# ACCtools/alignasm

Measured on AMD Instinct MI355X. Metric: contigs_per_sec, higher is better.
Workload: dtype int64

## Files before the change

alignasm_amd/_abi.py:

```python
import ctypes as C

import numpy as np

AASM_N_PHASES = 16
PHASE_NAMES = ["sort", "pairs", "edges", "revcsr", "sptree", "fwd", "heap", "enum", "select", "gather", "heap_prep", "topo", "misc", "cs", "final", "chain"]

AASM_OK = 0
AASM_E_INVAL, AASM_E_NODEVICE, AASM_E_HIP, AASM_E_NOMEM = -1, -2, -3, -4
AASM_E_OVERFLOW, AASM_E_INTERNAL, AASM_E_PARSE, AASM_E_IO = -5, -6, -7, -8

AASM_READ_DEVICE_RANGES, AASM_READ_H_WEAK_HASH, AASM_READ_H_FEW_BLOCKS = 1, 0x100, 0x200
AASM_READ_ROW_COLS, AASM_READ_TEXT_ON_DEVICE = 2, 4

DEBUG_POISON_SIG = (C.c_int, [C.c_int])

_IN_ARRAYS = [
    ("ctg_rec_off", np.int64), ("qry_str", np.int64), ("qry_end", np.int64), ("ref_str", np.int64),
    ("ref_end", np.int64), ("qry_total", np.int64), ("ref_chr", np.int32), ("aln_fwd", np.uint8),
    ("map_qul", np.uint8), ("rec_rng_off", np.int64), ("rng_qry_l", np.int64), ("rng_qry_r", np.int64),
    ("rng_ref_l", np.int64),
]


class BatchIn(C.Structure):
    _fields_ = [("n_contigs", C.c_int64), ("n_records", C.c_int64), ("n_ranges", C.c_int64)] + [
        (name, C.c_void_p) for name, _ in _IN_ARRAYS
    ] + [("cs_text", C.c_void_p), ("rec_cs_off", C.c_void_p)]


class Opts(C.Structure):
    _fields_ = [
        ("max_paths", C.c_int32), ("non_skip_linkable", C.c_int32), ("device", C.c_int32),
        ("collect_timing", C.c_int32), ("keep_debug", C.c_int32), ("reserved", C.c_int32 * 3),
    ]


AASM_H0_SEQ_SELECT, AASM_H0_HEAP_MW_ALL, AASM_H0_HEAP_MW_NONE, AASM_H0_ENUM_HEAP, AASM_H0_ENUM_SMALL = 0x1, 0x2, 0x4, 0x8, 0x10
AASM_H0_GRID_ORDER, AASM_H0_CHAIN_MASK, AASM_H0_CHAIN_ALL, AASM_H0_CHAIN_NONE, AASM_H0_CHAIN_HALF = 0x20, 0xC0, 0x40, 0x80, 0xC0
AASM_H0_MW_MASK, AASM_H0_MW_INPUT_ORDER, AASM_H0_MW_SHIFT, AASM_H0_GRAPH_LAUNCHES = 0xFF00, 1, 8, 0x10000
AASM_H2_LAUNCH_FAILURE, AASM_H2_WRAP_DEVICES, AASM_H2_DIRTY_SCAN, AASM_H2_CHAIN_HDR_LOST, AASM_H2_CHAIN_DONE_LOST = 0x1, 0x2, 0x4, 0x8, 0x10
AASM_H2_CHAIN_OWN_QUEUE, AASM_H2_SMALL_ROOT_RING, AASM_H2_SORT_DEPTH_MASK, AASM_H2_SORT_DEPTH_SHIFT = 0x20, 0x40, 0xFF00, 8
HOOK_CONSTANTS = {k: v for k, v in globals().items() if k.startswith(("AASM_H0_", "AASM_H2_"))}
_flag = lambda bits: {False: 0, True: bits}
HOOKS = {
    "sequential_select": (0, _flag(AASM_H0_SEQ_SELECT)), "heap_waves": (0, {"auto": 0, "all": AASM_H0_HEAP_MW_ALL, "none": AASM_H0_HEAP_MW_NONE}),
    "enum_heap": (0, _flag(AASM_H0_ENUM_HEAP)), "enum_small": (0, _flag(AASM_H0_ENUM_SMALL)), "grid_order": (0, _flag(AASM_H0_GRID_ORDER)),
    "chain": (0, {"auto": 0, "all": AASM_H0_CHAIN_ALL, "none": AASM_H0_CHAIN_NONE, "half": AASM_H0_CHAIN_HALF}),
    "heap_input_order": (0, _flag(AASM_H0_MW_INPUT_ORDER << AASM_H0_MW_SHIFT)), "heap_block_waves": (0, {n: n << AASM_H0_MW_SHIFT for n in (0, 4, 8, 16)}),
    "graph_launches": (0, _flag(AASM_H0_GRAPH_LAUNCHES)), "test_max_contigs": (1, None),
    "test_inject_launch_failure": (2, _flag(AASM_H2_LAUNCH_FAILURE)), "wrap_devices": (2, _flag(AASM_H2_WRAP_DEVICES)), "test_dirty_scan": (2, _flag(AASM_H2_DIRTY_SCAN)),
    "test_chain_lost": (2, {0: 0, 1: AASM_H2_CHAIN_HDR_LOST, 2: AASM_H2_CHAIN_DONE_LOST}), "chain_own_queue": (2, _flag(AASM_H2_CHAIN_OWN_QUEUE)),
    "test_small_root_ring": (2, _flag(AASM_H2_SMALL_ROOT_RING)), "sort_depth_test": (2, {d: d << AASM_H2_SORT_DEPTH_SHIFT for d in range(256)}),
}


def make_opts(max_paths=10000, non_skip_linkable=False, device=0, timing=False, keep_debug=False, **hooks):
    o = Opts(int(max_paths), 1 if non_skip_linkable else 0, int(device), 1 if timing else 0, 1 if keep_debug else 0)
    for name, value in hooks.items():
        if name not in HOOKS:
            raise TypeError(f"unknown test hook {name!r}")
        word, table = HOOKS[name]
        if table is not None and value not in table:
            raise ValueError(f"test hook {name}={value!r}: not one of {sorted(table, key=str)}")
        o.reserved[word] |= int(value) if table is None else table[value]
    if hooks.get("heap_input_order") and hooks.get("heap_block_waves"):
        raise ValueError("heap_input_order and heap_block_waves set the same field")
    return o


class OutElem(C.Structure):
    _fields_ = [
        ("edited_qry_str", C.c_int64), ("edited_qry_end", C.c_int64), ("edited_ref_str", C.c_int64),
        ("edited_ref_end", C.c_int64), ("ctg_index", C.c_int32), ("is_alt_path", C.c_int32),
    ]


OUT_ELEM_DTYPE = np.dtype(
    [("qs", np.int64), ("qe", np.int64), ("rs", np.int64), ("re", np.int64), ("ctg_index", np.int32), ("is_alt", np.int32)]
)

_STAT_I64 = [
    "n_vertices", "n_pairs", "n_edges", "n_heap_nodes", "n_paths_found", "n_paths_converted",
# ... 240 lines not shown
```

alignasm_amd/csrc/aasm_gpu.hip:

```cpp
#include <hip/hip_runtime.h>
#include <initializer_list>

#include <atomic>
#include <chrono>
#include <functional>
#include <mutex>
#include <thread>
#include <fcntl.h>
#include <sys/mman.h>
#include <sys/stat.h>
#include <unistd.h>

#include "aasm_pipeline.h"
#include "aasm_ksw.h"
#include "aasm_cut.h"
#include "aasm_read.h"
#include "aasm_rows.h"
#include "aasm_paf.hpp"

namespace aasm {

__device__ inline int64_t xcd_bid(int64_t b, int64_t g, int on) {
    if (!on || g < 64) return b;
    const int64_t g8 = g & ~(int64_t)7;
// ... 186 lines not shown
    for (int64_t base = 0; base < n; base += 4096) {
        const int64_t i0 = base + (int64_t)threadIdx.x * 4;
        int64_t va[4], vb[4], sa = 0, sb = 0;
#pragma unroll
        for (int i = 0; i < 4; i++) { va[i] = (i0 + i < n) ? (int64_t)in_a[i0 + i] : 0; sa += va[i]; vb[i] = (in_b && i0 + i < n) ? (int64_t)in_b[i0 + i] : 0; sb += vb[i]; }
        const int64_t ia = scan_wave_incl(sa, lane), ib = scan_wave_incl(sb, lane);
        if (lane == 63) { sh_w[0][wv] = ia; sh_w[1][wv] = ib; }
        __syncthreads();
        int64_t oa = sh_carry[0], ob = sh_carry[1], ta = 0, tb = 0;
#pragma unroll
        for (int i = 0; i < 16; i++) { const int64_t xa = sh_w[0][i], xb = sh_w[1][i]; if (i < wv) { oa += xa; ob += xb; } ta += xa; tb += xb; }
        int64_t ra = oa + ia - sa, rb = ob + ib - sb;
#pragma unroll
        for (int i = 0; i < 4; i++) { if (i0 + i < n) { out_a[i0 + i] = ra; if (in_b) out_b[i0 + i] = rb; } ra += va[i]; rb += vb[i]; }
        __syncthreads();
        if (threadIdx.x == 0) { sh_carry[0] += ta; sh_carry[1] += tb; }
        __syncthreads();
    }
    if (threadIdx.x == 0) { out_a[n] = sh_carry[0]; if (in_b) out_b[n] = sh_carry[1]; }
}

struct ScalarSrc { const int64_t *p[12]; };
__global__ void aasm_read_scalars(ScalarSrc src, int n, int64_t *dst) {
    const int i = (int)threadIdx.x;
    if (i < n) __hip_atomic_store(dst + i, *src.p[i], __ATOMIC_RELAXED, __HIP_MEMORY_SCOPE_SYSTEM);
}

struct ArenaBlock { char *p; size_t cap, used; };

struct DevCtx {
    int device = -1;
    bool ready = false;
    hipStream_t stream = nullptr, side = nullptr, side2 = nullptr;
    hipEvent_t ev_fork, ev_join, ev_fork2, ev_join2, ev_fork_b;
    int64_t *d_scratch2 = nullptr;
    size_t d_scratch2_cap = 0;
    std::vector<ArenaBlock> blocks;
    int64_t *pinned = nullptr;
    int64_t *pinned_dev = nullptr;
    char *stage[2] = {nullptr, nullptr};
    int64_t *d_scratch = nullptr;
    size_t d_scratch_cap = 0;
    uint64_t generation = 0;
    std::atomic<int> input_arrived{0};
    std::mutex mu;
    hipEvent_t ev_b[AASM_N_PHASES], ev_e[AASM_N_PHASES], ev_t0, ev_t1;
    int n_events_made = 0;
    int n_events2 = 0;
    hipEvent_t *timing_event(int i) { return i < AASM_N_PHASES ? &ev_b[i] : i < 2 * AASM_N_PHASES ? &ev_e[i - AASM_N_PHASES] : i == 2 * AASM_N_PHASES ? &ev_t0 : &ev_t1; }
    bool events = false;
    size_t peak_bytes = 0;
    std::vector<hipEvent_t> export_events;
};

static void drain_exports(DevCtx &cx) {
    for (hipEvent_t e : cx.export_events) { (void)hipEventSynchronize(e); (void)hipEventDestroy(e); }
    cx.export_events.clear();
}
static DevCtx g_ctx[16];
static std::mutex g_init_mu;
static std::atomic<int64_t> g_n_range_splits{0}, g_n_device_mallocs{0}, g_n_stream_syncs{0}, g_n_read_slow_rows{0}, g_n_read_fallbacks{0}, g_n_read_containers{0};

static std::atomic<int> g_poison{0};
static inline int poison_byte() { return g_poison.load(std::memory_order_relaxed); }

static std::string hip_err(const char *what, hipError_t e) {
    return std::string(what) + ": " + hipGetErrorString(e);
}

static int ctx_init(int device) {
    if (device < 0 || device >= 16) { set_last_error("device ordinal out of range"); return AASM_E_INVAL; }
    std::lock_guard<std::mutex> lk(g_init_mu);
    DevCtx &cx = g_ctx[device];
    if (cx.ready) return AASM_OK;
    int n = 0;
    hipError_t e = hipGetDeviceCount(&n);
    if (e != hipSuccess || n <= 0) { set_last_error("no HIP device available (this library has no CPU fallback)"); return AASM_E_NODEVICE; }
    if (device >= n) { set_last_error("device ordinal beyond hipGetDeviceCount"); return AASM_E_NODEVICE; }
    if ((e = hipSetDevice(device)) != hipSuccess) { set_last_error(hip_err("hipSetDevice", e)); return AASM_E_NODEVICE; }
    auto fail = [&](const char *what, hipError_t err) {
        set_last_error(hip_err(what, err));
        if (cx.pinned) { hipHostFree(cx.pinned); cx.pinned = nullptr; }
        if (cx.n_events_made > 0) { hipEventDestroy(cx.ev_fork); }
        if (cx.n_events_made > 1) { hipEventDestroy(cx.ev_join); }
        for (int i = 2; i < cx.n_events_made; i++) hipEventDestroy(*cx.timing_event(i - 2));
        cx.n_events_made = 0;
        if (cx.n_events2 > 0) { hipEventDestroy(cx.ev_fork2); }
        if (cx.n_events2 > 1) { hipEventDestroy(cx.ev_join2); }
        if (cx.n_events2 > 2) { hipEventDestroy(cx.ev_fork_b); }
        cx.n_events2 = 0;
        if (cx.side2) { hipStreamDestroy(cx.side2); cx.side2 = nullptr; }
        if (cx.side) { hipStreamDestroy(cx.side); cx.side = nullptr; }
        if (cx.stream) { hipStreamDestroy(cx.stream); cx.stream = nullptr; }
        return AASM_E_NODEVICE;
    };
    if ((e = hipStreamCreateWithFlags(&cx.stream, hipStreamNonBlocking)) != hipSuccess) return fail("hipStreamCreate", e);
    if ((e = hipStreamCreateWithFlags(&cx.side, hipStreamNonBlocking)) != hipSuccess) return fail("hipStreamCreate", e);
    if ((e = hipStreamCreateWithFlags(&cx.side2, hipStreamNonBlocking)) != hipSuccess) return fail("hipStreamCreate", e);
    if ((e = hipEventCreateWithFlags(&cx.ev_fork2, hipEventDisableTiming)) != hipSuccess) return fail("hipEventCreate", e);
    cx.n_events2 = 1;
    if ((e = hipEventCreateWithFlags(&cx.ev_join2, hipEventDisableTiming)) != hipSuccess) return fail("hipEventCreate", e);
    cx.n_events2 = 2;
    if ((e = hipEventCreateWithFlags(&cx.ev_fork_b, hipEventDisableTiming)) != hipSuccess) return fail("hipEventCreate", e);
    cx.n_events2 = 3;
    if ((e = hipEventCreateWithFlags(&cx.ev_fork, hipEventDisableTiming)) != hipSuccess) return fail("hipEventCreate", e);
    cx.n_events_made = 1;
    if ((e = hipEventCreateWithFlags(&cx.ev_join, hipEventDisableTiming)) != hipSuccess) return fail("hipEventCreate", e);
    cx.n_events_made = 2;
    for (int i = 0; i < 2 * AASM_N_PHASES + 2; i++) {
        if ((e = hipEventCreate(cx.timing_event(i))) != hipSuccess) return fail("hipEventCreate", e);
        cx.n_events_made++;
    }
    if ((e = hipHostMalloc((void **)&cx.pinned, 64 * sizeof(int64_t), hipHostMallocMapped)) != hipSuccess) return fail("hipHostMalloc", e);
    std::memset(cx.pinned, 0, 64 * sizeof(int64_t));
    if ((e = hipHostGetDevicePointer((void **)&cx.pinned_dev, cx.pinned, 0)) != hipSuccess) return fail("hipHostGetDevicePointer", e);
    cx.events = true;
    cx.device = device;
    cx.ready = true;
    return AASM_OK;
}

struct GpuBackend {
    static constexpr bool host_emulation = false;
    DevCtx &cx;
    hipStream_t stream, main_stream;
    bool on_side = false, forked = false, forked2 = false;
    bool timing;
    bool fail = false, out_of_memory = false;
    bool phase_used[AASM_N_PHASES] = {false};
    size_t cur_block = 0, bytes = 0;
    std::map<std::string, std::pair<void *, size_t>> named;
    GpuBackend(DevCtx &c, hipStream_t s, bool t) : cx(c), stream(s), main_stream(s), timing(t) {
        drain_exports(cx);
        for (auto &b : cx.blocks) b.used = 0;
        cx.generation++;
    }
    struct Attach {};
    GpuBackend(DevCtx &c, hipStream_t s, Attach) : cx(c), stream(s), main_stream(s), timing(false) {}
    void hip_fail(const char *what, hipError_t e) { if (!fail) set_last_error(hip_err(what, e)); fail = true; }
    void *alloc(const char *name, size_t n) {
        n = (n + 255) & ~(size_t)255;
        while (cur_block < cx.blocks.size() && cx.blocks[cur_block].used + n > cx.blocks[cur_block].cap) cur_block++;
        if (cur_block >= cx.blocks.size()) {
            size_t have = 0;
            for (auto &b : cx.blocks) have += b.cap;
            size_t cap = have > ((size_t)1 << 30) ? have : ((size_t)1 << 30);
            if (cap < n) cap = n;
            char *p = nullptr;
            hipError_t e = hipMalloc((void **)&p, cap);
            g_n_device_mallocs++;
            if (e == hipErrorOutOfMemory && cap > n) { (void)hipGetLastError(); cap = n; e = hipMalloc((void **)&p, cap); g_n_device_mallocs++; }
            if (e != hipSuccess) {
                if (e == hipErrorOutOfMemory) { (void)hipGetLastError(); out_of_memory = true; if (!fail) set_last_error("out of device memory (workspace arena)"); fail = true; }
                else hip_fail("hipMalloc", e);
                return nullptr;
            }
            cx.blocks.push_back(ArenaBlock{p, cap, 0});
            cur_block = cx.blocks.size() - 1;
            if (const int pz = poison_byte()) {
// ... 111 lines not shown
    int64_t read_i64(const int64_t *p) { int64_t v = 0; read_i64s({p}, &v); return v; }
    void read_i64s(std::initializer_list<const int64_t *> ps, int64_t *out) {
        int n = 0;
        for (auto p : ps) { (void)p; out[n++] = 0; }
        flush_zero();
        if (fail) return;
        ScalarSrc src;
        int i = 0;
        for (auto p : ps) { if (i < 12) src.p[i] = p; i++; }
        for (int j = i; j < 12; j++) src.p[j] = nullptr;
        hipLaunchKernelGGL(aasm_read_scalars, dim3(1), dim3(64), 0, stream, src, n, cx.pinned_dev);
        hipError_t e = hipGetLastError();
        if (e == hipSuccess) e = hipStreamSynchronize(stream);
        g_n_stream_syncs++;
        if (e != hipSuccess) { hip_fail("scalar read-back", e); return; }
        if (scan_stalled()) return;
        for (i = 0; i < n; i++) out[i] = cx.pinned[i];
    }
    void d2h(void *dst, const void *src, size_t n) {
        flush_zero();
        if (fail || n == 0) return;
        hipError_t e = hipMemcpyAsync(dst, src, n, hipMemcpyDeviceToHost, stream);
        if (e == hipSuccess) e = hipStreamSynchronize(stream);
        if (e != hipSuccess) hip_fail("hipMemcpy D2H", e);
        scan_stalled();
    }
    void h2d(void *dst, const void *src, size_t n) {
        flush_zero();
        if (fail || n == 0) return;
        hipError_t e = hipMemcpyAsync(dst, src, n, hipMemcpyHostToDevice, stream);
        if (e != hipSuccess) hip_fail("hipMemcpy H2D", e);
    }
    void fork() { flush_zero(); if (fail) return; hipEventRecord(cx.ev_fork, main_stream); hipStreamWaitEvent(cx.side, cx.ev_fork, 0); forked = true; }
    void fork_again() { flush_zero(); if (fail) return; hipEventRecord(cx.ev_fork_b, main_stream); hipStreamWaitEvent(cx.side, cx.ev_fork_b, 0); forked = true; }
    void use_side(bool on) { flush_zero(); on_side = on; stream = on ? cx.side : main_stream; }
    void join() { flush_zero(); if (fail || !forked) return; hipEventRecord(cx.ev_join, cx.side); hipStreamWaitEvent(main_stream, cx.ev_join, 0); forked = false; }
    void fork2() { flush_zero(); if (fail) return; hipEventRecord(cx.ev_fork2, main_stream); hipStreamWaitEvent(cx.side2, cx.ev_fork2, 0); forked2 = true; }
    void use_side2(bool on) { flush_zero(); stream = on ? cx.side2 : main_stream; }
    void join2() { flush_zero(); if (fail || !forked2) return; hipEventRecord(cx.ev_join2, cx.side2); hipStreamWaitEvent(main_stream, cx.ev_join2, 0); forked2 = false; }
    void phase_begin(int ph) { flush_zero(); if (timing && !fail) { hipError_t e = hipEventRecord(cx.ev_b[ph], stream); if (e != hipSuccess) hip_fail("hipEventRecord", e); phase_used[ph] = true; } }
    void phase_end(int ph) { flush_zero(); if (timing && !fail) { hipError_t e = hipEventRecord(cx.ev_e[ph], stream); if (e != hipSuccess) hip_fail("hipEventRecord", e); } }
};

struct GraphGpu {
    hipStream_t stream;
    const char *entry;
    hipError_t e = hipSuccess;
    std::vector<void *> blocks;
    ~GraphGpu() { for (void *p : blocks) hipFree(p); }
    void *alloc(size_t n) {
        void *p = nullptr;
        if (e != hipSuccess) return nullptr;
        if ((e = hipMalloc(&p, n)) != hipSuccess) { (void)hipGetLastError(); return nullptr; }
        blocks.push_back(p);
        if (const int pz = poison_byte()) { if ((e = hipMemsetAsync(p, pz, n, stream)) != hipSuccess) return nullptr; }
        return p;
    }
    size_t mark() const { return blocks.size(); }
    void release(size_t m) { while (blocks.size() > m) { hipFree(blocks.back()); blocks.pop_back(); } }
    bool h2d(void *d, const void *h, size_t n) { return e == hipSuccess && (e = hipMemcpyAsync(d, h, n, hipMemcpyHostToDevice, stream)) == hipSuccess; }
    bool fill(void *d, int byte, size_t n) { return e == hipSuccess && (e = hipMemsetAsync(d, byte, n, stream)) == hipSuccess; }
    bool d2h(void *h, const void *d, size_t n) {
        if (e == hipSuccess) e = hipMemcpyAsync(h, d, n, hipMemcpyDeviceToHost, stream);
        return sync();
    }
    bool sync() { return e == hipSuccess && (e = hipStreamSynchronize(stream)) == hipSuccess; }
    bool launched() { return e == hipSuccess && (e = hipGetLastError()) == hipSuccess; }
    bool launch_from(int kid, int64_t g0, int64_t g1, const KswArgs &a) {
        if (e != hipSuccess) return false;
// ... 1185 lines not shown
```

alignasm_amd/csrc/aasm_kernels.h:

```cpp
#pragma once
#include <cstddef>
#include "aasm_dev.h"
#include "../../include/alignasm_amd.h"

namespace aasm {

struct PqK;
struct WS {
    int64_t C, R, R0, S, VT, ET;
    int32_t K, nsl;
    int32_t avg_sidetracks;
    int32_t xcd_map;
    int32_t mw_compact;
    int32_t sort_depth_test;
    const int64_t *rec_off, *in_qs, *in_qe, *in_rs, *in_re, *in_qt, *in_rng_off, *rql, *rqr, *rrl;
    const int32_t *in_chr;
    const uint8_t *in_fwd, *in_mq;
    const char *cs_text;
    const int64_t *cs_off;
    int64_t *rng_rec;
    int64_t rng_stride;
    int32_t *cs_bad;
    int32_t *perm, *dupflag, *np, *pstart;
    int64_t *s_qs, *s_qe, *s_rs, *s_re, *s_qt, *s_rb;
// ... 18 lines not shown
    int64_t *hoff;
    int32_t *hcap_cnt;
    HNode *hnodes;
    int32_t *h_root, *bq, *h_cnt;
    Dist *kd;
    int32_t *klast, *kfound;
    I4 *kcand;
    PqK *pq;
    int64_t pq_stride;
    int32_t *pathA, *pathB, *pathT, *pre2, *stamp;
    Dist *dist2;
    uint8_t *notalt;
    int32_t *mark_time;
    int32_t *plan_kk;
    int32_t *nconv, *cv_ctg, *cv_k, *cv_ord, *cv_kind, *cv_szr, *cv_szv, *cv_n, *cv_err, *cv_path, *cv_pre2, *cv_stamp, *cv_la;
    int64_t *conv_off, *cv_roff, *cv_voff, *cv_cov;
    OutElem *cv_out;
    Dist *cv_dist2;
    int64_t NCONV;
    OutElem *cur_out, *main_out, *alt_out, *pool;
    int32_t *main_len, *alt_len, *all_gen, *all_seq;
    int32_t *ar_ctg, *ar_gen, *ar_seq, *ar_len;
    int64_t *ar_off;
    int64_t pool_cap, ar_cap;
    int64_t *main_off, *alt_off;
    OutElem *main_c, *alt_c;
    int32_t *status;
    int64_t *counters;
    int32_t *gb_flag; int32_t gb_off;
    int64_t *prof_heap, *prof_sel, *prof_gb;
    Dist *st_cost;
    int32_t *st_n;
    I4 *vhdr, *vhdr2, *cinfo;
    int32_t mw_mode;
    int32_t *mw_flag, *mw_lg;
    HNode *hprov;
    int64_t *mw_off;
    int32_t *mw_cap;
    int32_t *mw_order, *mw_rs, *mw_fb;
    int32_t *mw_rsv, *mw_used;
    int32_t *mw_list, *mw_sorted;
    int32_t *mw_key;
    int32_t mw_n, mw_base;
    I4 *tnx;
    int32_t *tnx16;
    I4 *rvh;
    I4 *r_pk;
    I4 *fvh;
    int32_t chain_mode;
    int32_t chain_all, chain_minN;
    int32_t chain_test;
    int32_t *chain_flag, *chain_list;
    int32_t *pend;
    int32_t *cq;
    I4 *bfsq;
    int32_t chain_ord;
    int32_t chain_rn;
};

enum { CNT_RANGE_STEPS = 0, CNT_UNCONN, CNT_POOL, CNT_AR, CNT_CONVERTED, CNT_HEAPNODES, CNT_PATHS, CNT_OVF, CNT_ISPR_E, CNT_ISPR_V, CNT_PATH_E, CNT_OUT_E, CNT_PQ_PUSH, CNT_MW, CNT_MAXN, CNT_LONGSORT, CNT_MAXV, CNT_CHAIN, CNT_GB_S, CNT_GB_L, CNT_GB_REST, CNT_N };

AASM_DEV void set_status(const WS &w, int64_t c, int code) { if (w.status[c] == 0) w.status[c] = code; }
AASM_DEV bool in_chain_class(const WS &w, int64_t c) { return w.chain_flag != nullptr && w.chain_flag[c] != 0; }
AASM_DEV bool in_graph_class(const WS &w, int64_t c) { return w.gb_flag && w.gb_flag[c] != 0; }
#define AASM_COORD_LIMIT ((int64_t)1 << 40)
AASM_DEV bool coord_ok(int64_t x) { return x >= 0 && x < AASM_COORD_LIMIT; }
// ... 2116 lines not shown
        n.q2.z = leaf ? eu : old.q2.z; n.q2.w = leaf ? ev : old.q2.w;
#if defined(AASM_HOST_EMUL)
        nodeq_store(&hs.ring[ni & (hs.rn - 1)], n);
        sp.n.at(j) = n; sp.idx.at(j) = ni; if (leaf) sp.sum.at(j) = ksum;
        if (!leaf && sw) swm |= 1ull << j;
#else
        if (in) {
            nodeq_store(&hs.ring[ni & (hs.rn - 1)], n);
            sp.n.at(j) = n; sp.idx.at(j) = ni; if (leaf) sp.sum.at(j) = ksum;
        }
        swm = wave_ballot(in && !leaf && sw);
#endif
    }
    if (swm) { const int t = ffs64(swm) - 1; sp.len = t + 1; sp.tail = LA_GET(sp.n, t, .q2.y); }
    else { sp.len = depth + 1; sp.tail = -1; }
    sp.root = alloc + depth;
    hs.alloc = nalloc;
    return sp.root;
}

struct KProfNone { int64_t acc[8]; };
AASM_DEV bool chain_wait_hdr(ChainSync *S, const I4 *vh, const I4 *vh2, int32_t u, int64_t patience) {
    const int64_t t0 = wave_realtime();
    int64_t guard = 0;
    for (;;) {
        const int32_t pd = uni(ld_shared_i32(&S->prep_done));
        const int32_t x = uni(ld_shared_i32(&vh[u].x)), y = uni(ld_shared_i32(&vh2[u].y));
        if (x != -1 && y != -1) { wave_fence(); return true; }
        if (pd) return false;
        if ((++guard & 1023) == 0 && wave_realtime() - t0 > patience) return false;
        wave_sleep();
    }
}
template <bool CHAIN = false, int RING = HEAP_RING_1W, int QN = HEAP_QN_1W>
AASM_DEV void kb_heap(const KCtx &k, const WS &w, ChainSync *S = nullptr) {
    const int64_t c = k.bid;
    const int64_t V = w.ctgV[c];
    if (V == 0) return;
    if (!CHAIN && in_chain_class(w, c)) return;
    HeapLdsT<RING, QN> *L = (HeapLdsT<RING, QN> *)k.lds;
    const int64_t vb = w.voff[c];
    int32_t *h = w.h_root + vb, *q = w.bq + vb;
    const I4 *vh = w.vhdr + vb, *vh2 = w.vhdr2 + vb;
    const Dist *sk = w.st_cost + w.rowptr[vb];
    HeapState hs;
    hs.nodes = w.hnodes + w.hoff[c]; hs.ring = L->ring; hs.rn = RING; hs.bounce = &L->bounce; hs.oldn = L->oldn; hs.alloc = 0; hs.flushed = 0; hs.ring_lo = 0; hs.ovf = false;
    hs.cap = (int32_t)(w.hoff[c + 1] - w.hoff[c]);
    const int32_t src = (int32_t)(V - 2), dest = (int32_t)(V - 1);
    if (w.mw_flag[c]) return;
#if !defined(AASM_HOST_EMUL)
    {
        const int64_t I = (w.rowptr[vb + V] - w.rowptr[vb]) - (V - 1);
        const int64_t a = w.avg_sidetracks > 0 ? w.avg_sidetracks : 1;
        if (8 * I > 9 * a) __builtin_amdgcn_s_setprio(3);
        else if (I > a) __builtin_amdgcn_s_setprio(2);
        else if (8 * I > 7 * a) __builtin_amdgcn_s_setprio(1);
    }
#endif
    if (k.lane == 0) w.h_cnt[c] = 0;
    if (w.status[c] != 0) return;
    if (!CHAIN && dist_is_max(w.sp_d[vb + src])) { if (k.lane == 0) set_status(w, c, -6); return; }
    bool chain_lost = false;
    const int64_t patience = (CHAIN && w.chain_test == 2) ? (int64_t)100000000 : (int64_t)30 * 100000000;
    int32_t head = 0, tail = 0, lds_hi = 0;
    Spine sp; sp.root = -2; sp.len = 0; sp.tail = -1;
#if defined(AASM_KPROF) && !defined(AASM_HOST_EMUL)
    KPROF_DECL;
    KPROF_START();
    struct KP { int64_t &t0; int64_t *acc; } kp{kp_t0, kp_acc};
#else
    KProfNone kp;
#endif
    int32_t u = dest, hu = -1, so = 0, n = 0;
    if (CHAIN && !chain_wait_hdr(S, vh, vh2, dest, patience)) chain_lost = true;
    else {
        const I4 a0 = vh[dest];
        so = uni(a0.x); n = uni(a0.y);
    }
    wave_lds_sync();
    int32_t pend_u = -1, pend_root = -1;
    int32_t staged = -1;
    int32_t c_nch = 0, c_fc = -1, c_sofc = 0, c_nfc = 0, c_c0lo = 0, c_c0hi = 0, c_n = 0;
    while (!hs.ovf && !chain_lost) {
        HeapStage *St = &L->stage;
        if (staged != u) {
            if (CHAIN && !chain_wait_hdr(S, vh, vh2, u, patience)) { chain_lost = true; break; }
            const I4 ha = vh[u], hb = vh2[u];
            so = uni(ha.x); c_n = uni(ha.y);
            FOR_LANE(t, (c_n < HEAP_KMAX ? c_n : HEAP_KMAX), k.lane) { const Dist kk = sk[(int64_t)so + t]; St->key[t] = kk; }
            c_nch = uni(ha.z); c_fc = uni(ha.w); c_sofc = uni(hb.z); c_nfc = uni(hb.w); c_c0lo = uni(hb.x); c_c0hi = uni(hb.y);
            wave_lds_sync();
        }
        n = c_n;
// ... 1792 lines not shown
```

alignasm_amd/csrc/aasm_pipeline.h:

```cpp
#pragma once
#include <algorithm>
#include <cstdlib>
#include <cstring>
#include <map>
#include <string>
#include <vector>

#include "../../include/alignasm_amd.h"
#include "aasm_kernels.h"
#include "aasm_enum.h"

namespace aasm {

enum Kern {
#define AASM_PIPELINE_KERNELS(K, KL)                                                                                                  \
    K(KN_CS_RANGES, aasm_k0_cs_ranges, 256, ALL_LANES, kb_cs_ranges)                                                                  \
    KL(KN_SORT, aasm_k1_sort, 256, 1, AASM_SORT_LDS_BYTES, 2, kb_sort)                                                                \
    K(KN_SORT_RANK, aasm_k1_sort_rank, 256, ALL_LANES, kb_sort_rank)                                                                  \
    KL(KN_SORT_FIX, aasm_k1_sort_fix, AASM_WAVE, 1, AASM_SORTFIX_LDS_BYTES, 1, kb_sort_fix)                                           \
    K(KN_GATHER_PARTS, aasm_k1_gather_parts, AASM_WAVE, 1, kb_gather_parts)                                                           \
    K(KN_OV_COUNT, aasm_k2_ov_count, 256, ALL_LANES, kb_ov_count)                                                                     \
    K(KN_OV_MERGE, aasm_k2_ov_merge, 256, ALL_LANES, kb_ov_merge)                                                                     \
    K(KN_VCOUNT, aasm_k2_vcount, 256, ALL_LANES, kb_vcount)                                                                           \
    K(KN_VFILL_REC, aasm_k2_vfill_rec, 256, ALL_LANES, kb_vfill_rec)                                                                  \
// ... 41 lines not shown
    K(KN_SEL_CLASSIFY, aasm_k9_sel_classify, 256, ALL_LANES, kb_sel_classify)                                                         \
    KL(KN_SEL_CONVERT, aasm_k9_sel_convert, AASM_WAVE, 1, AASM_SEL_LDS_BYTES, 5, kb_sel_convert)                                      \
    K(KN_SEL_FINAL, aasm_k9_sel_final, AASM_WAVE, 1, kb_sel_final)                                                                    \
            \
    KL(KN_CHAIN, aasm_k67_chain, AASM_WAVE * CHAIN_WAVES, CHAIN_WAVES, AASM_CHAIN_LDS_BYTES, 5, kb_chain<true>)                       \
                 \
    KL(KN_CHAIN3, aasm_k67_chain3, AASM_WAVE * (CHAIN_WAVES - 1), CHAIN_WAVES - 1, AASM_CHAIN_LDS_BYTES, 5, kb_chain<false>)          \
    K(KN_K7_PREP, aasm_k7_prep, 256, ALL_LANES, kb_k7_prep)                                                                           \
    K(KN_TNX, aasm_k9_tnx, 256, ALL_LANES, kb_tnx)                                                                                    \
    K(KN_TNX16, aasm_k9_tnx16, 256, ALL_LANES, kb_tnx16)                                                                              \
                                                                  \
    KL(KN_TNX16_WG, aasm_k9_tnx16_wg, TNX_TPB, 1, AASM_TNXWG_LDS_BYTES, 4, kb_tnx16_wg)
    AASM_PIPELINE_KERNELS(AASM_ROW_ID, AASM_ROW_ID)
};
constexpr int kern_block[] = {AASM_PIPELINE_KERNELS(AASM_ROW_BLOCK, AASM_ROW_BLOCK)};
AASM_KERNEL_BODY(run_kernel_body, AASM_PIPELINE_KERNELS, WS)

template <class B> void launch(B &be, int kn, int64_t nblocks, const WS &w) { be.launch(kn, nblocks, kern_block[kn], w); }

static inline int64_t cdiv(int64_t a, int64_t b) { return (a + b - 1) / b; }
#ifndef AASM_CHAIN_ORD_MAX
#define AASM_CHAIN_ORD_MAX 1024
#endif
#define AASM_CHAIN_SMALL_BATCH 1536

#ifndef AASM_GROUPED_MIN
#define AASM_GROUPED_MIN 2560
#endif
struct PipelineSizes { int64_t C = 0, R = 0, S = 0, VT = 0, ET = 0, HT = 0, bad_record = -1; };

struct Hooks {
    bool seq_select, enum_heap, enum_small, grid_order, graph_launches, chain_half, launch_failure, wrap_devices, dirty_scan, chain_own_queue;
    int32_t heap_mw, chain, chain_test, root_ring, sort_depth;
    int32_t mw;
    int64_t range_limit;
};
static inline Hooks decode_hooks(const aasm_opts &o) {
    const int32_t h0 = o.reserved[0], h2 = o.reserved[2], ch = h0 & AASM_H0_CHAIN_MASK;
    Hooks h;
    h.seq_select = h0 & AASM_H0_SEQ_SELECT; h.enum_heap = h0 & AASM_H0_ENUM_HEAP; h.enum_small = h0 & AASM_H0_ENUM_SMALL;
    h.grid_order = h0 & AASM_H0_GRID_ORDER; h.graph_launches = h0 & AASM_H0_GRAPH_LAUNCHES; h.chain_half = ch == AASM_H0_CHAIN_HALF;
    h.heap_mw = (h0 & AASM_H0_HEAP_MW_ALL) ? 1 : (h0 & AASM_H0_HEAP_MW_NONE) ? 2 : 0;
    h.chain = ch == AASM_H0_CHAIN_ALL ? 1 : ch == AASM_H0_CHAIN_NONE ? 2 : 0;
    h.mw = (h0 & AASM_H0_MW_MASK) >> AASM_H0_MW_SHIFT; h.range_limit = o.reserved[1];
    h.launch_failure = h2 & AASM_H2_LAUNCH_FAILURE; h.wrap_devices = h2 & AASM_H2_WRAP_DEVICES; h.dirty_scan = h2 & AASM_H2_DIRTY_SCAN;
    h.chain_test = (h2 & AASM_H2_CHAIN_DONE_LOST) ? 2 : (h2 & AASM_H2_CHAIN_HDR_LOST) ? 1 : 0; h.chain_own_queue = h2 & AASM_H2_CHAIN_OWN_QUEUE;
    h.root_ring = (h2 & AASM_H2_SMALL_ROOT_RING) ? 4 : 0; h.sort_depth = (h2 & AASM_H2_SORT_DEPTH_MASK) >> AASM_H2_SORT_DEPTH_SHIFT;
    return h;
}

struct FormSizes { int64_t C, R, K, VT, ET, MAXV, NCHAIN, HTM, NMW, MAXN; };
struct Forms {
    bool grouped, dense, mw_ranked;
    int rev_fill, chain, mw_kern, enum_kern;
};
static inline Forms choose_forms(const FormSizes &s, const Hooks &h, bool host_emulation) {
    Forms f;
    f.dense = s.ET > 6 * s.VT;
    f.grouped = !f.dense && s.C >= AASM_GROUPED_MIN;
    f.rev_fill = f.dense && s.MAXV <= REV_ORD_MAXV ? (s.MAXV <= REV_ORD_MIDV ? KN_REV_FILL_ORD_S : KN_REV_FILL_ORD) : f.dense ? KN_REV_FILL_W : KN_REV_FILL;
    f.chain = !h.chain_own_queue && s.NCHAIN <= AASM_CHAIN_ORD_MAX ? KN_CHAIN : KN_CHAIN3;
    const int mw_waves = (h.mw == 4 || h.mw == 8 || h.mw == 16) ? h.mw : s.NMW * 16 <= 6144 ? 16 : s.NMW * 8 <= 6144 ? 8 : 4;
    f.mw_kern = mw_waves == 16 ? KN_HEAP_MW16 : mw_waves == 8 ? KN_HEAP_MW8 : KN_HEAP_MW;
    f.mw_ranked = h.mw != AASM_H0_MW_INPUT_ORDER && s.NMW >= 2 && s.NMW <= 32768;
    const bool enum_heap = host_emulation || h.enum_heap || s.MAXN > AASM_ENUM_MAX_N;
    f.enum_kern = enum_heap ? KN_ENUM_HEAP : ((s.C > 14 * 256 && s.C <= 20 * 256 && s.K > 21) || h.enum_small) ? KN_ENUM_S : KN_ENUM;
    return f;
}

template <class B>
int run_pipeline(B &be, const aasm_batch_in &in, const aasm_opts &opts, WS &w, PipelineSizes &sz) {
    std::memset(&w, 0, sizeof(w));
    const int64_t C = in.n_contigs;
    int64_t rr[2];
    be.read_i64s({in.ctg_rec_off, in.ctg_rec_off + C}, rr);
    const int64_t R0 = rr[0], R1 = rr[1];
    const int64_t R = R1 - R0;
    w.C = C; w.R = R; w.R0 = R0;
    w.K = opts.max_paths > 0 ? opts.max_paths : 10000;
    w.nsl = opts.non_skip_linkable ? 1 : 0;
    const Hooks h = decode_hooks(opts);
    w.xcd_map = h.grid_order ? 0 : 1; w.sort_depth_test = h.sort_depth;
    w.chain_mode = h.chain; w.chain_test = h.chain_test; w.chain_rn = h.root_ring;
    w.chain_ord = h.chain_own_queue ? 0 : 1;
    w.chain_all = (!h.chain_half && C <= AASM_CHAIN_SMALL_BATCH) ? 1 : 0;
    w.chain_minN = (int32_t)std::min<int64_t>(std::max<int64_t>(2048, 4 * (R / std::max<int64_t>(C, 1))), INT32_MAX);
    if (h.chain_half) w.chain_minN = (int32_t)std::min<int64_t>(std::max<int64_t>(1, cdiv(R, std::max<int64_t>(C, 1))), INT32_MAX);
    w.rec_off = in.ctg_rec_off; w.in_qs = in.qry_str; w.in_qe = in.qry_end; w.in_rs = in.ref_str; w.in_re = in.ref_end;
    w.in_qt = in.qry_total; w.in_chr = in.ref_chr; w.in_fwd = in.aln_fwd; w.in_mq = in.map_qul;
    w.in_rng_off = in.rec_rng_off; w.rql = in.rng_qry_l; w.rqr = in.rng_qry_r; w.rrl = in.rng_ref_l; w.rng_stride = 1;
    sz.C = C; sz.R = R;
    if (C <= 0 || R <= 0) return AASM_E_INVAL;
// ... 146 lines not shown
            be.phase_begin(AASM_PH_FWD);
            if (f.grouped) launch(be, KN_FWD_SWEEP_G, cdiv(C, sweep_n), w);
            else launch(be, KN_FWD_SWEEP, C, w);
            be.phase_end(AASM_PH_FWD);
            be.phase_begin(AASM_PH_TOPO);
            launch(be, KN_TOPO_COUNT, cdiv(VT, 256), w);
            be.scan_i32(w.tp_deg, VT, w.tp_ptr);
            launch(be, KN_TOPO_FILL, cdiv(VT, AASM_WAVE), w);
            be.phase_end(AASM_PH_TOPO);
            be.use_side(false);
        };
        side_work();
        A(ccnt, int32_t, VT, "ccnt"); A(cval, int32_t, ET, "cval");
        A(st_cost, Dist, ET, "st_cost"); A(st_n, int32_t, VT, "st_n"); A(vhdr, I4, VT, "vhdr"); A(vhdr2, I4, VT, "vhdr2"); A(cinfo, I4, ET, "cinfo"); A(tnx, I4, VT, "tnx"); A(tnx16, int32_t, 16 * VT, "tnx16");
        sz.HT = HT;
        w.avg_sidetracks = (int32_t)std::min<int64_t>((ET - VT + C) / (C > 0 ? C : 1), INT32_MAX);
        A(hnodes, HNode, HT, "hnodes"); A(h_root, int32_t, VT, "h_root"); A(bq, int32_t, VT, "bq");
        A(hprov, HNode, HTM, "hprov");
        A(mw_order, int32_t, VT, "mw_order"); A(mw_rs, int32_t, VT, "mw_rs"); A(mw_fb, int32_t, VT, "mw_fb"); A(mw_rsv, int32_t, VT, "mw_rsv"); A(mw_used, int32_t, VT, "mw_used");
        CHECK_ALLOC();
        be.fill_ff(w.h_root, sizeof(int32_t) * (size_t)VT);
        be.fill_ff(w.bq, sizeof(int32_t) * (size_t)VT);
        if (NCHAIN > 0) {
            be.fill_ff(w.vhdr, sizeof(I4) * (size_t)VT);
            be.fill_ff(w.vhdr2, sizeof(I4) * (size_t)VT);
            be.fork2();
            be.use_side2(true);
            be.phase_begin(AASM_PH_CHAIN);
            if (f.chain == KN_CHAIN) launch(be, KN_CHAIN, NCHAIN, w);
            else launch(be, KN_CHAIN3, NCHAIN, w);
            be.phase_end(AASM_PH_CHAIN);
            be.use_side2(false);
        }
        if (NCHAIN < C) {
        be.phase_begin(AASM_PH_SPTREE);
        if (f.grouped) launch(be, KN_REV_SWEEP_G, cdiv(C, sweep_n), w);
        else launch(be, KN_REV_SWEEP, C, w);
        be.phase_end(AASM_PH_SPTREE);

        be.fork_again();
        be.use_side(true);
        if (GB_S + GB_L > 0) launch(be, KN_TNX16_WG, C, w);
        if (GB_REST > 0) {
            launch(be, KN_TNX, cdiv(VT, 256), w);
            launch(be, KN_TNX16, cdiv(VT, 256), w);
        }
        be.use_side(false);
        be.phase_begin(AASM_PH_HEAP_PREP);
        if (f.dense) {
            launch(be, KN_CHILDREN, cdiv(VT, 256), w);
            launch(be, KN_SIDETRACK_W, cdiv(VT, AASM_WAVE), w);
            launch(be, KN_HEAP_HDR, cdiv(VT, 256), w);
        } else launch(be, KN_K7_PREP, cdiv(VT, 256), w);
        be.phase_end(AASM_PH_HEAP_PREP);
        be.join();
        be.phase_begin(AASM_PH_HEAP);
        launch(be, KN_HEAP, C, w);
        w.mw_n = (int32_t)NMW; w.mw_base = -1;
        if (HTM > 0) {
            if (f.mw_ranked) {
                launch(be, KN_MW_RANK, cdiv(NMW, 256), w);
                w.mw_base = 0;
                { const int32_t xm = w.xcd_map; w.xcd_map = 0; launch(be, f.mw_kern, NMW, w); w.xcd_map = xm; }
                w.mw_base = -1;
            } else launch(be, f.mw_kern, C, w);
        }
        be.phase_end(AASM_PH_HEAP);
        }
        be.join2();

        const int64_t K = w.K;
        A(kd, Dist, C * K, "kd"); A(klast, int32_t, C * K, "klast");
        w.pq_stride = f.enum_kern == KN_ENUM_HEAP ? 3 * K + 1 : enum_stride(K);
        A(kcand, I4, 2 * C * (3 * K + 1), "kcand"); A(pq, PqK, C * w.pq_stride, "pq");
        CHECK_ALLOC();
        be.phase_begin(AASM_PH_ENUM);
        launch(be, f.enum_kern, C, w);
        be.phase_end(AASM_PH_ENUM);
    }

    be.join();
    A(mark_time, int32_t, R, "mark_time");
    A(conv_off, int64_t, C + 1, "conv_off"); A(plan_kk, int32_t, C * 2 * SEL_PLAN_KEEP, "plan_kk");
    CHECK_ALLOC();
    be.fill_byte(w.mark_time, 0x7F, sizeof(int32_t) * (size_t)R);
    bool sequential = h.seq_select;
    int64_t NCONV = 0, SR = 0, SV = 0;
    bool nm_ready = false;
    int64_t nm[2] = {0, 0};
    if (!sequential) {
        be.phase_begin(AASM_PH_MISC);
        if (VT > 0) launch(be, KN_SEL_PLAN, C, w);
        be.scan_i32(w.nconv, C, w.conv_off);
        NCONV = be.read_i64(w.conv_off + C);
        w.NCONV = NCONV;
        if (NCONV > 0) {
            A(cv_ctg, int32_t, NCONV, "cv_ctg"); A(cv_k, int32_t, NCONV, "cv_k"); A(cv_ord, int32_t, NCONV, "cv_ord"); A(cv_kind, int32_t, NCONV, "cv_kind");
            A(cv_szr, int32_t, NCONV, "cv_szr"); A(cv_szv, int32_t, NCONV, "cv_szv"); A(cv_roff, int64_t, NCONV + 1, "cv_roff"); A(cv_voff, int64_t, NCONV + 1, "cv_voff");
            AZ(cv_n, int32_t, NCONV, "cv_n"); AZ(cv_err, int32_t, NCONV, "cv_err"); AZ(cv_cov, int64_t, NCONV, "cv_cov"); A(cv_la, int32_t, NCONV, "cv_la");
            CHECK_ALLOC();
            launch(be, KN_SEL_PLANFILL, C, w);
            be.scan_i32_pair(w.cv_szr, w.cv_roff, w.cv_szv, w.cv_voff, NCONV);
// ... 241 lines not shown
```

include/alignasm_amd.h:

```cpp
#ifndef ALIGNASM_AMD_H
#define ALIGNASM_AMD_H

#include <stdint.h>

#ifdef __cplusplus
extern "C" {
#endif

#define AASM_ABI_VERSION 3

#define AASM_OK              0
#define AASM_E_INVAL        -1
#define AASM_E_NODEVICE     -2
#define AASM_E_HIP          -3
#define AASM_E_NOMEM        -4
#define AASM_E_OVERFLOW     -5
#define AASM_E_INTERNAL     -6
#define AASM_E_PARSE        -7
#define AASM_E_IO           -8

typedef struct aasm_batch_in {
    int64_t n_contigs;
    int64_t n_records;
    int64_t n_ranges;
// ... 16 lines not shown

typedef struct aasm_opts {
    int32_t max_paths;
    int32_t non_skip_linkable;
    int32_t device;
    int32_t collect_timing;
    int32_t keep_debug;
    int32_t reserved[3];
} aasm_opts;

#define AASM_H0_SEQ_SELECT       0x1
#define AASM_H0_HEAP_MW_ALL      0x2
#define AASM_H0_HEAP_MW_NONE     0x4
#define AASM_H0_ENUM_HEAP        0x8
#define AASM_H0_ENUM_SMALL       0x10
#define AASM_H0_GRID_ORDER       0x20
#define AASM_H0_CHAIN_MASK       0xC0
#define AASM_H0_CHAIN_ALL        0x40
#define AASM_H0_CHAIN_NONE       0x80
#define AASM_H0_CHAIN_HALF       0xC0
#define AASM_H0_MW_MASK          0xFF00
#define AASM_H0_MW_INPUT_ORDER   1
#define AASM_H0_MW_SHIFT         8
#define AASM_H0_GRAPH_LAUNCHES   0x10000
#define AASM_H2_LAUNCH_FAILURE   0x1
#define AASM_H2_WRAP_DEVICES     0x2
#define AASM_H2_DIRTY_SCAN       0x4
#define AASM_H2_CHAIN_HDR_LOST   0x8
#define AASM_H2_CHAIN_DONE_LOST  0x10
#define AASM_H2_CHAIN_OWN_QUEUE  0x20
#define AASM_H2_SMALL_ROOT_RING  0x40
#define AASM_H2_SORT_DEPTH_MASK  0xFF00
#define AASM_H2_SORT_DEPTH_SHIFT 8

typedef struct aasm_out_elem {
    int64_t edited_qry_str, edited_qry_end;
    int64_t edited_ref_str, edited_ref_end;
    int32_t ctg_index;
    int32_t is_alt_path;
} aasm_out_elem;

#define AASM_N_PHASES 16
typedef struct aasm_stats {
    int64_t n_vertices;
    int64_t n_pairs;
    int64_t n_edges;
    int64_t n_heap_nodes;
    int64_t n_paths_found;
    int64_t n_paths_converted;
    int64_t n_unconnectable;
    int64_t n_internal_errors;
    int64_t n_single;
    int64_t range_steps;
    int64_t device_bytes;
    int64_t ispr_edges;
    int64_t ispr_vertices;
    int64_t path_edges;
    int64_t out_elems;
    int64_t pq_pushes;
    float   phase_ms[AASM_N_PHASES];
    float   total_ms;
    float   reserved_f[3];
} aasm_stats;

enum {
    AASM_PH_SORT = 0,
// ... 222 lines not shown
```

Measured before the change: 447,400.

## Defer sparse jump-record kernels past heap and add optional in-heap prep pass

For sparse graphs, the jump-record (TNX) kernels are now forked onto the side stream after the heap phase rather than before heap prep. This lets them overlap with enumeration instead of competing with heap prep and heap building. An opt-in hook fuses the children, sidetrack and header prep into the start of the heap kernel, replacing the separate K7 prep launch. A dedicated join event is added for the second fork. The deferred fork risks less overlap if enumeration is short.

Result: no change. 449,000 (median of 2 runs) (+0.4%).

```diff
diff --git a/alignasm_amd/_abi.py b/alignasm_amd/_abi.py
--- a/alignasm_amd/_abi.py
+++ b/alignasm_amd/_abi.py
@@ -41,13 +41,16 @@
 AASM_H2_LAUNCH_FAILURE, AASM_H2_WRAP_DEVICES, AASM_H2_DIRTY_SCAN, AASM_H2_CHAIN_HDR_LOST, AASM_H2_CHAIN_DONE_LOST = 0x1, 0x2, 0x4, 0x8, 0x10
 AASM_H2_CHAIN_OWN_QUEUE, AASM_H2_SMALL_ROOT_RING, AASM_H2_SORT_DEPTH_MASK, AASM_H2_SORT_DEPTH_SHIFT = 0x20, 0x40, 0xFF00, 8
 HOOK_CONSTANTS = {k: v for k, v in globals().items() if k.startswith(("AASM_H0_", "AASM_H2_"))}
+AASM_H0_PREP_LAUNCH, AASM_H0_PREP_IN_HEAP = 0x20000, 0x40000
+HOOK_ENUMERATORS = {"AASM_H0_PREP_LAUNCH": AASM_H0_PREP_LAUNCH, "AASM_H0_PREP_IN_HEAP": AASM_H0_PREP_IN_HEAP}
 _flag = lambda bits: {False: 0, True: bits}
 HOOKS = {
     "sequential_select": (0, _flag(AASM_H0_SEQ_SELECT)), "heap_waves": (0, {"auto": 0, "all": AASM_H0_HEAP_MW_ALL, "none": AASM_H0_HEAP_MW_NONE}),
     "enum_heap": (0, _flag(AASM_H0_ENUM_HEAP)), "enum_small": (0, _flag(AASM_H0_ENUM_SMALL)), "grid_order": (0, _flag(AASM_H0_GRID_ORDER)),
     "chain": (0, {"auto": 0, "all": AASM_H0_CHAIN_ALL, "none": AASM_H0_CHAIN_NONE, "half": AASM_H0_CHAIN_HALF}),
     "heap_input_order": (0, _flag(AASM_H0_MW_INPUT_ORDER << AASM_H0_MW_SHIFT)), "heap_block_waves": (0, {n: n << AASM_H0_MW_SHIFT for n in (0, 4, 8, 16)}),
-    "graph_launches": (0, _flag(AASM_H0_GRAPH_LAUNCHES)), "test_max_contigs": (1, None),
+    "graph_launches": (0, _flag(AASM_H0_GRAPH_LAUNCHES)), "prep_launch": (0, {True: AASM_H0_PREP_LAUNCH, False: AASM_H0_PREP_IN_HEAP}),
+    "test_max_contigs": (1, None),
     "test_inject_launch_failure": (2, _flag(AASM_H2_LAUNCH_FAILURE)), "wrap_devices": (2, _flag(AASM_H2_WRAP_DEVICES)), "test_dirty_scan": (2, _flag(AASM_H2_DIRTY_SCAN)),
     "test_chain_lost": (2, {0: 0, 1: AASM_H2_CHAIN_HDR_LOST, 2: AASM_H2_CHAIN_DONE_LOST}), "chain_own_queue": (2, _flag(AASM_H2_CHAIN_OWN_QUEUE)),
     "test_small_root_ring": (2, _flag(AASM_H2_SMALL_ROOT_RING)), "sort_depth_test": (2, {d: d << AASM_H2_SORT_DEPTH_SHIFT for d in range(256)}),
diff --git a/alignasm_amd/csrc/aasm_gpu.hip b/alignasm_amd/csrc/aasm_gpu.hip
--- a/alignasm_amd/csrc/aasm_gpu.hip
+++ b/alignasm_amd/csrc/aasm_gpu.hip
@@ -242,7 +242,7 @@
     int device = -1;
     bool ready = false;
     hipStream_t stream = nullptr, side = nullptr, side2 = nullptr;
-    hipEvent_t ev_fork, ev_join, ev_fork2, ev_join2, ev_fork_b;
+    hipEvent_t ev_fork, ev_join, ev_fork2, ev_join2, ev_fork_b, ev_join_b;
     int64_t *d_scratch2 = nullptr;
     size_t d_scratch2_cap = 0;
     std::vector<ArenaBlock> blocks;
@@ -298,6 +298,7 @@
         if (cx.n_events2 > 0) { hipEventDestroy(cx.ev_fork2); }
         if (cx.n_events2 > 1) { hipEventDestroy(cx.ev_join2); }
         if (cx.n_events2 > 2) { hipEventDestroy(cx.ev_fork_b); }
+        if (cx.n_events2 > 3) { hipEventDestroy(cx.ev_join_b); }
         cx.n_events2 = 0;
         if (cx.side2) { hipStreamDestroy(cx.side2); cx.side2 = nullptr; }
         if (cx.side) { hipStreamDestroy(cx.side); cx.side = nullptr; }
@@ -313,6 +314,8 @@
     cx.n_events2 = 2;
     if ((e = hipEventCreateWithFlags(&cx.ev_fork_b, hipEventDisableTiming)) != hipSuccess) return fail("hipEventCreate", e);
     cx.n_events2 = 3;
+    if ((e = hipEventCreateWithFlags(&cx.ev_join_b, hipEventDisableTiming)) != hipSuccess) return fail("hipEventCreate", e);
+    cx.n_events2 = 4;
     if ((e = hipEventCreateWithFlags(&cx.ev_fork, hipEventDisableTiming)) != hipSuccess) return fail("hipEventCreate", e);
     cx.n_events_made = 1;
     if ((e = hipEventCreateWithFlags(&cx.ev_join, hipEventDisableTiming)) != hipSuccess) return fail("hipEventCreate", e);
@@ -334,7 +337,7 @@
     static constexpr bool host_emulation = false;
     DevCtx &cx;
     hipStream_t stream, main_stream;
-    bool on_side = false, forked = false, forked2 = false;
+    bool on_side = false, forked = false, forked2 = false, forked_again = false;
     bool timing;
     bool fail = false, out_of_memory = false;
     bool phase_used[AASM_N_PHASES] = {false};
@@ -512,9 +515,15 @@
         if (e != hipSuccess) hip_fail("hipMemcpy H2D", e);
     }
     void fork() { flush_zero(); if (fail) return; hipEventRecord(cx.ev_fork, main_stream); hipStreamWaitEvent(cx.side, cx.ev_fork, 0); forked = true; }
-    void fork_again() { flush_zero(); if (fail) return; hipEventRecord(cx.ev_fork_b, main_stream); hipStreamWaitEvent(cx.side, cx.ev_fork_b, 0); forked = true; }
+    void fork_again() { flush_zero(); if (fail) return; hipEventRecord(cx.ev_fork_b, main_stream); hipStreamWaitEvent(cx.side, cx.ev_fork_b, 0); forked = true; forked_again = true; }
     void use_side(bool on) { flush_zero(); on_side = on; stream = on ? cx.side : main_stream; }
-    void join() { flush_zero(); if (fail || !forked) return; hipEventRecord(cx.ev_join, cx.side); hipStreamWaitEvent(main_stream, cx.ev_join, 0); forked = false; }
+    void join() {
+        flush_zero();
+        if (fail || !forked) return;
+        hipEvent_t ev = forked_again ? cx.ev_join_b : cx.ev_join;
+        hipEventRecord(ev, cx.side); hipStreamWaitEvent(main_stream, ev, 0);
+        forked = false; forked_again = false;
+    }
     void fork2() { flush_zero(); if (fail) return; hipEventRecord(cx.ev_fork2, main_stream); hipStreamWaitEvent(cx.side2, cx.ev_fork2, 0); forked2 = true; }
     void use_side2(bool on) { flush_zero(); stream = on ? cx.side2 : main_stream; }
     void join2() { flush_zero(); if (fail || !forked2) return; hipEventRecord(cx.ev_join2, cx.side2); hipStreamWaitEvent(main_stream, cx.ev_join2, 0); forked2 = false; }
diff --git a/alignasm_amd/csrc/aasm_kernels.h b/alignasm_amd/csrc/aasm_kernels.h
--- a/alignasm_amd/csrc/aasm_kernels.h
+++ b/alignasm_amd/csrc/aasm_kernels.h
@@ -74,6 +74,7 @@
     Dist *st_cost;
     int32_t *st_n;
     I4 *vhdr, *vhdr2, *cinfo;
+    int32_t heap_prep;
     int32_t mw_mode;
     int32_t *mw_flag, *mw_lg;
     HNode *hprov;
@@ -2256,12 +2257,26 @@
         wave_sleep();
     }
 }
+AASM_DEV void heap_prepass(const KCtx &k, const WS &w, int64_t c, int64_t V) {
+    const int64_t vb = w.voff[c];
+    for (int64_t v = k.tid; v < V; v += k.nthreads) {
+        const int64_t gv = vb + v;
+        int32_t ch4[4];
+        const int32_t nch = children_vertex(w, gv, ch4);
+        const int32_t nkeys = sidetrack_vertex(w, gv);
+        I4 a, b;
+        heap_hdr_vertex(w, gv, a, b, nch, ch4, nkeys);
+        w.vhdr[gv] = a; w.vhdr2[gv] = b;
+    }
+    wave_fence();
+}
 template <bool CHAIN = false, int RING = HEAP_RING_1W, int QN = HEAP_QN_1W>
 AASM_DEV void kb_heap(const KCtx &k, const WS &w, ChainSync *S = nullptr) {
     const int64_t c = k.bid;
     const int64_t V = w.ctgV[c];
     if (V == 0) return;
     if (!CHAIN && in_chain_class(w, c)) return;
+    if (!CHAIN && w.heap_prep) heap_prepass(k, w, c, V);
     HeapLdsT<RING, QN> *L = (HeapLdsT<RING, QN> *)k.lds;
     const int64_t vb = w.voff[c];
     int32_t *h = w.h_root + vb, *q = w.bq + vb;
@@ -2282,7 +2297,7 @@
     }
 #endif
     if (k.lane == 0) w.h_cnt[c] = 0;
-    if (w.status[c] != 0) return;
+    if ((CHAIN ? w.status[c] : uni(ld_shared_i32(&w.status[c]))) != 0) return;
     if (!CHAIN && dist_is_max(w.sp_d[vb + src])) { if (k.lane == 0) set_status(w, c, -6); return; }
     bool chain_lost = false;
     const int64_t patience = (CHAIN && w.chain_test == 2) ? (int64_t)100000000 : (int64_t)30 * 100000000;
diff --git a/alignasm_amd/csrc/aasm_pipeline.h b/alignasm_amd/csrc/aasm_pipeline.h
--- a/alignasm_amd/csrc/aasm_pipeline.h
+++ b/alignasm_amd/csrc/aasm_pipeline.h
@@ -97,6 +97,7 @@
 struct Hooks {
     bool seq_select, enum_heap, enum_small, grid_order, graph_launches, chain_half, launch_failure, wrap_devices, dirty_scan, chain_own_queue;
     int32_t heap_mw, chain, chain_test, root_ring, sort_depth;
+    int32_t heap_prep;
     int32_t mw;
     int64_t range_limit;
 };
@@ -104,7 +105,7 @@
     const int32_t h0 = o.reserved[0], h2 = o.reserved[2], ch = h0 & AASM_H0_CHAIN_MASK;
     Hooks h;
     h.seq_select = h0 & AASM_H0_SEQ_SELECT; h.enum_heap = h0 & AASM_H0_ENUM_HEAP; h.enum_small = h0 & AASM_H0_ENUM_SMALL;
-    h.grid_order = h0 & AASM_H0_GRID_ORDER; h.graph_launches = h0 & AASM_H0_GRAPH_LAUNCHES; h.chain_half = ch == AASM_H0_CHAIN_HALF;
+    h.grid_order = h0 & AASM_H0_GRID_ORDER; h.graph_launches = h0 & AASM_H0_GRAPH_LAUNCHES; h.heap_prep = (h0 & AASM_H0_PREP_LAUNCH) ? 2 : (h0 & AASM_H0_PREP_IN_HEAP) ? 1 : 0; h.chain_half = ch == AASM_H0_CHAIN_HALF;
     h.heap_mw = (h0 & AASM_H0_HEAP_MW_ALL) ? 1 : (h0 & AASM_H0_HEAP_MW_NONE) ? 2 : 0;
     h.chain = ch == AASM_H0_CHAIN_ALL ? 1 : ch == AASM_H0_CHAIN_NONE ? 2 : 0;
     h.mw = (h0 & AASM_H0_MW_MASK) >> AASM_H0_MW_SHIFT; h.range_limit = o.reserved[1];
@@ -117,12 +118,14 @@
 struct FormSizes { int64_t C, R, K, VT, ET, MAXV, NCHAIN, HTM, NMW, MAXN; };
 struct Forms {
     bool grouped, dense, mw_ranked;
+    bool heap_prep;
     int rev_fill, chain, mw_kern, enum_kern;
 };
 static inline Forms choose_forms(const FormSizes &s, const Hooks &h, bool host_emulation) {
     Forms f;
     f.dense = s.ET > 6 * s.VT;
     f.grouped = !f.dense && s.C >= AASM_GROUPED_MIN;
+    f.heap_prep = !f.dense && h.heap_prep == 1;
     f.rev_fill = f.dense && s.MAXV <= REV_ORD_MAXV ? (s.MAXV <= REV_ORD_MIDV ? KN_REV_FILL_ORD_S : KN_REV_FILL_ORD) : f.dense ? KN_REV_FILL_W : KN_REV_FILL;
     f.chain = !h.chain_own_queue && s.NCHAIN <= AASM_CHAIN_ORD_MAX ? KN_CHAIN : KN_CHAIN3;
     const int mw_waves = (h.mw == 4 || h.mw == 8 || h.mw == 16) ? h.mw : s.NMW * 16 <= 6144 ? 16 : s.NMW * 8 <= 6144 ? 8 : 4;
@@ -335,29 +338,37 @@
             be.phase_end(AASM_PH_CHAIN);
             be.use_side2(false);
         }
+        auto jump_records = [&]() {
+            be.fork_again();
+            be.use_side(true);
+            if (GB_S + GB_L > 0) launch(be, KN_TNX16_WG, C, w);
+            if (GB_REST > 0) {
+                launch(be, KN_TNX, cdiv(VT, 256), w);
+                launch(be, KN_TNX16, cdiv(VT, 256), w);
+            }
+            be.use_side(false);
+        };
         if (NCHAIN < C) {
         be.phase_begin(AASM_PH_SPTREE);
         if (f.grouped) launch(be, KN_REV_SWEEP_G, cdiv(C, sweep_n), w);
         else launch(be, KN_REV_SWEEP, C, w);
         be.phase_end(AASM_PH_SPTREE);
 
-        be.fork_again();
-        be.use_side(true);
-        if (GB_S + GB_L > 0) launch(be, KN_TNX16_WG, C, w);
-        if (GB_REST > 0) {
-            launch(be, KN_TNX, cdiv(VT, 256), w);
-            launch(be, KN_TNX16, cdiv(VT, 256), w);
-        }
-        be.use_side(false);
-        be.phase_begin(AASM_PH_HEAP_PREP);
         if (f.dense) {
+            jump_records();
+            be.phase_begin(AASM_PH_HEAP_PREP);
             launch(be, KN_CHILDREN, cdiv(VT, 256), w);
             launch(be, KN_SIDETRACK_W, cdiv(VT, AASM_WAVE), w);
             launch(be, KN_HEAP_HDR, cdiv(VT, 256), w);
-        } else launch(be, KN_K7_PREP, cdiv(VT, 256), w);
-        be.phase_end(AASM_PH_HEAP_PREP);
+            be.phase_end(AASM_PH_HEAP_PREP);
+        } else if (!f.heap_prep) {
+            be.phase_begin(AASM_PH_HEAP_PREP);
+            launch(be, KN_K7_PREP, cdiv(VT, 256), w);
+            be.phase_end(AASM_PH_HEAP_PREP);
+        }
         be.join();
         be.phase_begin(AASM_PH_HEAP);
+        w.heap_prep = f.heap_prep ? 1 : 0;
         launch(be, KN_HEAP, C, w);
         w.mw_n = (int32_t)NMW; w.mw_base = -1;
         if (HTM > 0) {
@@ -371,6 +382,7 @@
         be.phase_end(AASM_PH_HEAP);
         }
         be.join2();
+        if (NCHAIN < C && !f.dense) jump_records();
 
         const int64_t K = w.K;
         A(kd, Dist, C * K, "kd"); A(klast, int32_t, C * K, "klast");
diff --git a/include/alignasm_amd.h b/include/alignasm_amd.h
--- a/include/alignasm_amd.h
+++ b/include/alignasm_amd.h
@@ -72,6 +72,10 @@
 #define AASM_H2_SMALL_ROOT_RING  0x40
 #define AASM_H2_SORT_DEPTH_MASK  0xFF00
 #define AASM_H2_SORT_DEPTH_SHIFT 8
+enum {
+    AASM_H0_PREP_LAUNCH  = 0x20000,
+    AASM_H0_PREP_IN_HEAP = 0x40000
+};
 
 typedef struct aasm_out_elem {
     int64_t edited_qry_str, edited_qry_end;
```
